# aimi-lab/robust-pose-estimator

Measured on AMD Instinct MI355X. Metric: stereo-pair pose solves/sec (640x512, 8 solver iters), higher is better.
Workload: dtype f32 (RAFT / geometry) + f64 (SE(3) solve), as the reference; 1 GPU; PoseNet.infer, 640x512 stereo frame pairs, 16 per GPU per step (RAFT batch 32), 12 GRU iters, lbfgs x8 SE(3) solve, weight heads on; frames_per_gpu=16, height=512, width=640, raft_iters=12, solver=lbfgs, solver_iters=8, parallelism=frames sharded x1

## Files before the change

### robust-pose-estimator_amd/csrc/conv_wino1d.hip

```cpp
#include "wino_common.h"
#include <type_traits>
#include <cstdlib>

#define W1_CO 64
#define W1_NT 64
#define W1_K 4
#define W1_ROW 8
#define W1_USTEP (W1_K * W1_CO * W1_ROW)
#define W1_RAWF 1536
#define W1_BIAS 1024u

struct W1P {
    const float* x; long long xbs;
    const float* wp; int cin, cout, coP, H, W;
    const float* bias; const float* add; long long abs_;
    float* out; long long obs; float* out2; long long o2bs;
    const float* hid; long long hbs; const float* z; long long zbs;
    int cgate, mode;
    int Hv, Wv;
};

__device__ __forceinline__ int row_swap(int r) { return ((r >> 2) ^ (r >> 3)) & 1; }

template <bool VERT, int CB, bool VALID = false>
__global__ __launch_bounds__(256, 2) void k_conv_wino1d(W1P P) {
    constexpr int TCO = 32 * CB, UT_STEP = W1_K * TCO * W1_ROW;
    __shared__ __attribute__((aligned(16))) float Us[3][UT_STEP];
    __shared__ __attribute__((aligned(16))) float Vs[2][W1_USTEP];
    __shared__ __attribute__((aligned(16))) float Rs[3][W1_RAWF];
    asm volatile("" :: "s"(P.x), "s"(P.wp), "s"(P.out), "s"(P.bias), "s"(P.xbs), "s"(P.obs), "s"(P.cin), "s"(P.cout), "s"(P.coP), "s"(P.H),
                 "s"(P.W), "s"(P.mode), "s"(P.cgate));
    asm volatile("" :: "s"(P.add), "s"(P.abs_), "s"(P.out2), "s"(P.o2bs), "s"(P.hid), "s"(P.hbs), "s"(P.z), "s"(P.zbs));
    const int tid = threadIdx.x, lane = tid & 63, wv = __builtin_amdgcn_readfirstlane(tid >> 6);
    const int ptx = (P.W + 15) / 16;
#ifndef WINO_NO_XCD
    const int pid = (gridDim.x & 7) == 0 ? (int)(blockIdx.x & 7) * (int)(gridDim.x >> 3) + (int)(blockIdx.x >> 3) : (int)blockIdx.x;
#else
    const int pid = blockIdx.x;
#endif
    const int x0 = (pid % ptx) * 16, y0 = (pid / ptx) * 16;
    const int co0 = blockIdx.y * TCO, bz = blockIdx.z;
    const int H = P.H, W = P.W, hw = H * W;
    const float* xb = P.x + (size_t)bz * P.xbs;
    const int nsteps = P.cin / W1_K;

    constexpr int LANES = VERT ? 40 : 48, RQ_CI = VERT ? 80 : 96, RQ_ROW = VERT ? 4 : 6;
    constexpr unsigned RSTRIDE = LANES * 16u;
    unsigned roff[2] = {0u, 0u};
    unsigned oob = 0;
    if (lane < LANES) {
#pragma unroll
        for (int j = 0; j < 2; ++j) {
            const int q = LANES * (2 * wv + j) + lane;
            const int ci = q / RQ_CI, rem = q - ci * RQ_CI, r = rem / RQ_ROW, cq = rem - r * RQ_ROW;
            int yy = VERT ? y0 - 2 + r : y0 + r, xx = VERT ? x0 + 4 * cq : x0 - 4 + 4 * cq;
            if (yy < 0 || yy >= H || xx < 0 || xx >= W) oob |= 1u << j;
            yy = yy < 0 ? 0 : (yy >= H ? H - 1 : yy); xx = xx < 0 ? 0 : (xx >= W ? W - 4 : xx);
            roff[j] = (unsigned)(ci * hw + yy * W + xx) * 4u + W1_BIAS - RSTRIDE * j;
        }
    }
    const bool border = VERT ? ((y0 < 2) | (y0 + 18 > H) | (x0 + 16 > W)) : ((y0 + 16 > H) | (x0 < 4) | (x0 + 20 > W));
    auto patch_raw = [&](int buf) {
        if (border) {
#pragma unroll
            for (int j = 0; j < 2; ++j)
                if ((oob >> j) & 1) *(f32x4*)&Rs[buf][4 * (LANES * (2 * wv + j) + lane)] = (f32x4){0.0f, 0.0f, 0.0f, 0.0f};
        }
    };
    const float* wslice = CB == 2 ? P.wp + (size_t)(co0 / W1_CO) * W1_USTEP + (size_t)(wv * 2) * 256
                                  : P.wp + (size_t)(co0 / W1_CO) * W1_USTEP + (size_t)wv * (W1_CO * W1_ROW) + (size_t)(co0 % W1_CO) * W1_ROW;
    const unsigned uoff = lane * 16u;
    const size_t wstep = (size_t)(P.coP / W1_CO) * W1_USTEP, rstep = (size_t)W1_K * hw;
    const unsigned us_base = lds_addr_of(&Us[0][0]) + (unsigned)wv * (CB == 2 ? 2048u : 1024u), rs_base = lds_addr_of(&Rs[0][0]) + (unsigned)(2 * wv) * RSTRIDE;
    const unsigned long long lane_mask = (1ull << LANES) - 1ull;
    auto dma_u = [&](const float* src, int buf) {
        if (CB == 2) dma16x2(src, uoff, us_base + (unsigned)buf * (UT_STEP * 4u));
        else dma16x1(src, uoff, us_base + (unsigned)buf * (UT_STEP * 4u));
    };
    auto dma_raw = [&](const float* src, int buf) { dma16x2_masked<RSTRIDE>(src, roff[0], roff[1], rs_base + (unsigned)buf * (W1_RAWF * 4u), lane_mask); };
    auto clamped = [&](int step) { return step < nsteps ? step : nsteps - 1; };
    const float* xsrc = xb - W1_BIAS / 4;

    const int t_src = VERT ? wv * (RQ_CI * 4) + (4 * (lane >> 4)) * 16 + (lane & 15) : wv * (RQ_CI * 4) + (lane >> 2) * 24 + 4 * (lane & 3) + 2;
    const int t_dst = (wv * W1_NT + lane) * W1_ROW, t_swap = row_swap(lane & 15);
    float d[8];
    f32x4 vlo, vhi;
    auto tr_read = [&](int rbuf) {
        const float* rp = &Rs[rbuf][t_src];
        if (VERT) {
#pragma unroll
            for (int k = 0; k < 8; ++k) d[k] = rp[16 * k];
        } else {
#pragma unroll
            for (int k = 0; k < 8; k += 2) { const float2 v = *(const float2*)(rp + k); d[k] = v.x; d[k + 1] = v.y; }
        }
    };
    auto tr_math = [&]() {
        const float a12 = fmaf(-4.25f, d[4], d[2] + d[6]), b12 = fmaf(-4.25f, d[3], d[1] + d[5]);
        const float a34 = fmaf(-1.25f, d[4], fmaf(0.25f, d[2], d[6])), b34 = fmaf(2.0f, d[5], fmaf(-2.5f, d[3], 0.5f * d[1]));
        const float a56 = fmaf(-5.0f, d[4], fmaf(4.0f, d[2], d[6])), b56 = fmaf(0.5f, d[5], fmaf(-2.5f, d[3], 2.0f * d[1]));
        vlo = (f32x4){fmaf(5.25f, d[4] - d[2], d[0] - d[6]), a12 + b12, a12 - b12, a34 + b34};
        vhi = (f32x4){a34 - b34, a56 + b56, a56 - b56, fmaf(5.25f, d[3] - d[5], d[7] - d[1])};
    };
    auto tr_store = [&](int vbuf) {
        *(f32x4*)&Vs[vbuf][t_dst + 4 * t_swap] = vlo;
        *(f32x4*)&Vs[vbuf][t_dst + 4 * (t_swap ^ 1)] = vhi;
    };

    f32x4 acc[8][CB][2];
#pragma unroll
    for (int p = 0; p < 8; ++p)
#pragma unroll
        for (int c = 0; c < CB; ++c)
#pragma unroll
            for (int t = 0; t < 2; ++t) acc[p][c][t] = (f32x4){0.0f, 0.0f, 0.0f, 0.0f};
    const int cw = wv >> 1, tw = wv & 1, li = lane & 15, lk = lane >> 4;
    float bi_[CB][4];
#pragma unroll
    for (int cb = 0; cb < CB; ++cb)
#pragma unroll
        for (int r = 0; r < 4; ++r) {
            const int co = co0 + cw * 16 * CB + cb * 16 + 4 * lk + r;
            bi_[cb][r] = P.bias ? P.bias[co < P.cout ? co : P.cout - 1] : 0.0f;
        }

    dma_u(wslice, 0); dma_raw(xsrc, 0); dma_raw(xsrc + (size_t)clamped(1) * rstep, 1);
    dma_u(wslice + (size_t)clamped(1) * wstep, 1); dma_raw(xsrc + (size_t)clamped(2) * rstep, 2);
    dma_u(wslice + (size_t)clamped(2) * wstep, 2);
    if (CB == 2) __builtin_amdgcn_s_waitcnt(0x0F76); else __builtin_amdgcn_s_waitcnt(0x0F74);
    patch_raw(0); patch_raw(1);
    __builtin_amdgcn_s_waitcnt(0xC07F);
    __builtin_amdgcn_s_barrier();
    tr_read(0); tr_math(); tr_store(0);
    __builtin_amdgcn_s_waitcnt(0xC07F);
    __builtin_amdgcn_s_barrier();
    dma_raw(xsrc + (size_t)clamped(3) * rstep, 0);
    const float* unext = wave_uniform(wslice + (size_t)clamped(3) * wstep);
    const float* rnext = wave_uniform(xsrc + (size_t)clamped(4) * rstep);
    const int sl = 4 * row_swap(li);
    const int aoff = (lk * TCO + cw * 16 * CB + li) * W1_ROW, boff = (lk * W1_NT + tw * 32 + li) * W1_ROW;
    f32x4 fa = *(const f32x4*)&Us[0][aoff + sl], fb0 = *(const f32x4*)&Vs[0][boff + sl], fb1 = *(const f32x4*)&Vs[0][boff + 16 * W1_ROW + sl];
    auto mfma_range = [&](int p0, int np, int cb, const f32x4& a, const f32x4& b0, const f32x4& b1) {
#pragma unroll
        for (int e = 0; e < np; ++e) {
            const int p = p0 + e;
            acc[p][cb][0] = __builtin_amdgcn_mfma_f32_16x16x4f32(a[p & 3], b0[p & 3], acc[p][cb][0], 0, 0, 0);
            acc[p][cb][1] = __builtin_amdgcn_mfma_f32_16x16x4f32(a[p & 3], b1[p & 3], acc[p][cb][1], 0, 0, 0);
        }
    };
    auto step = [&](auto ubc, auto curc, const int s) {
        constexpr int UB = decltype(ubc)::value, CUR = decltype(curc)::value, UB1 = (UB + 1) % 3, UB2 = (UB + 2) % 3;
        const float* ua = &Us[UB][aoff];
        const float* vb = &Vs[CUR][boff];
        f32x4 a_lo1 = fa;
        if (CB == 2) a_lo1 = *(const f32x4*)(ua + 16 * W1_ROW + sl);
        tr_read(UB1);
        __builtin_amdgcn_sched_barrier(0);
        if (CB == 2) mfma_range(0, 4, 0, fa, fb0, fb1); else mfma_range(0, 2, 0, fa, fb0, fb1);
        __builtin_amdgcn_sched_barrier(0);
        const f32x4 a_hi0 = *(const f32x4*)(ua + (sl ^ 4)), b_hi0 = *(const f32x4*)(vb + (sl ^ 4)), b_hi1 = *(const f32x4*)(vb + 16 * W1_ROW + (sl ^ 4));
        __builtin_amdgcn_sched_barrier(0);
        tr_math();
        __builtin_amdgcn_sched_barrier(0);
        if (CB == 2) mfma_range(0, 4, CB - 1, a_lo1, fb0, fb1); else mfma_range(2, 2, 0, fa, fb0, fb1);
        __builtin_amdgcn_sched_barrier(0);
        f32x4 a_hi1 = a_hi0;
        if (CB == 2) a_hi1 = *(const f32x4*)(ua + 16 * W1_ROW + (sl ^ 4));
        __builtin_amdgcn_sched_barrier(0);
        tr_store(CUR ^ 1);
        __builtin_amdgcn_sched_barrier(0);
        if (CB == 2) mfma_range(4, 4, 0, a_hi0, b_hi0, b_hi1); else mfma_range(4, 2, 0, a_hi0, b_hi0, b_hi1);
        __builtin_amdgcn_sched_barrier(0);
        if (CB == 2) __builtin_amdgcn_s_waitcnt(0x0F74); else __builtin_amdgcn_s_waitcnt(0x0F73);
        patch_raw(UB2);
        __builtin_amdgcn_s_waitcnt(0xC07F);
        __builtin_amdgcn_s_barrier();
        __builtin_amdgcn_sched_barrier(0);
        fa = *(const f32x4*)&Us[UB1][aoff + sl]; fb0 = *(const f32x4*)&Vs[CUR ^ 1][boff + sl]; fb1 = *(const f32x4*)&Vs[CUR ^ 1][boff + 16 * W1_ROW + sl];
        __builtin_amdgcn_sched_barrier(0);
#pragma unroll
        for (int e = 0; e < 2 * CB; ++e) {
            const int p = CB == 2 ? 4 + e : 6 + e;
            acc[p][CB - 1][0] = __builtin_amdgcn_mfma_f32_16x16x4f32(a_hi1[p & 3], b_hi0[p & 3], acc[p][CB - 1][0], 0, 0, 0);
            acc[p][CB - 1][1] = __builtin_amdgcn_mfma_f32_16x16x4f32(a_hi1[p & 3], b_hi1[p & 3], acc[p][CB - 1][1], 0, 0, 0);
            __builtin_amdgcn_sched_barrier(0);
            if (e == 0) { dma_u(unext, UB); if (s + 4 < nsteps) unext += wstep; }
            if (e == 1) { dma_raw(rnext, UB1); if (s + 5 < nsteps) rnext += rstep; }
            __builtin_amdgcn_sched_barrier(0);
        }
    };
    {
        typedef std::integral_constant<int, 0> I0; typedef std::integral_constant<int, 1> I1; typedef std::integral_constant<int, 2> I2;
        int s = 0;
        while (true) {
            step(I0{}, I0{}, s); if (++s == nsteps) break;
            step(I1{}, I1{}, s); if (++s == nsteps) break;
            step(I2{}, I0{}, s); if (++s == nsteps) break;
            step(I0{}, I1{}, s); if (++s == nsteps) break;
            step(I1{}, I0{}, s); if (++s == nsteps) break;
            step(I2{}, I1{}, s); if (++s == nsteps) break;
        }
    }
    __builtin_amdgcn_s_waitcnt(0x0F70);

    const int mode = P.mode, cg = P.cgate;
    const float* addb = P.add ? P.add + (size_t)bz * P.abs_ : nullptr;
    const float* hb = P.hid ? P.hid + (size_t)bz * P.hbs : nullptr;
    const float* zb = P.z ? P.z + (size_t)bz * P.zbs : nullptr;
    float* outb = P.out + (size_t)bz * P.obs;
    float* out2b = P.out2 ? P.out2 + (size_t)bz * P.o2bs : nullptr;
    float* tsc = &Us[0][wv * (CB == 2 ? 512 : 256)] + lk * 64;
    auto epilogue = [&](auto modec, auto fastc) {
        constexpr int MODE = decltype(modec)::value;
        constexpr bool FAST = decltype(fastc)::value;
        const bool rtile = co0 >= cg;
        constexpr int NB = 4 * CB, RU = 2;
        const f32x4 zero4 = {0.0f, 0.0f, 0.0f, 0.0f};
        auto where = [&](int tb, int& oy, int& ox) {
            const int tile = tw * 32 + tb * 16 + li;
            oy = VERT ? y0 + 4 * (tile >> 4) + (li >> 2) : y0 + (tile >> 2); ox = VERT ? x0 + 4 * (li & 3) : x0 + 4 * (tile & 3);
        };
        auto load_block = [&](int n, f32x4 (&av)[RU], f32x4 (&xv)[RU], f32x4 (&hv)[RU]) {
            const int tb = (n >> 1) / CB, cb = (n >> 1) % CB, r0 = RU * (n & 1);
            int oy, ox; where(tb, oy, ox);
            const bool pok = FAST || ((oy < H) & (ox < W));
            const size_t pxo = (size_t)oy * W + ox;
#pragma unroll
            for (int q = 0; q < RU; ++q) {
                const int co = co0 + cw * 16 * CB + cb * 16 + 4 * lk + r0 + q;
                const bool ok = FAST || (pok && co < P.cout);
                const size_t e0 = (size_t)co * hw + pxo;
                av[q] = (addb && ok) ? *(const f32x4*)(addb + e0) : zero4;
                xv[q] = hv[q] = zero4;
                if (MODE == RPE_CONV_GATE_ZR) { if (FAST ? rtile : (ok && co >= cg)) xv[q] = *(const f32x4*)(hb + e0 - (size_t)cg * hw); }
                else if (MODE == RPE_CONV_GATE_H) { if (ok) { xv[q] = *(const f32x4*)(zb + e0); hv[q] = *(const f32x4*)(hb + e0); } }
            }
        };
        auto finish_block = [&](int n, const f32x4 (&av)[RU], const f32x4 (&xv)[RU], const f32x4 (&hv)[RU]) {
            const int tb = (n >> 1) / CB, cb = (n >> 1) % CB, r0 = RU * (n & 1);
            int oy, ox; where(tb, oy, ox);
            const bool pok = FAST || ((oy < H) & (ox < W));
            const size_t pxo = (size_t)oy * W + ox;
            auto st4 = [&](float* p, size_t e, const float (&v)[4]) {
                f32x4 q4 = {v[0], v[1], v[2], v[3]};
                if (VALID && !FAST) {
#pragma unroll
                    for (int i = 0; i < 4; ++i) q4[i] = (oy < P.Hv && ox + i < P.Wv) ? q4[i] : 0.0f;
                }
                if (pok) *(f32x4*)(p + e) = q4;
            };
#pragma unroll
            for (int q = 0; q < RU; ++q) {
                const int r = r0 + q, co = co0 + cw * 16 * CB + cb * 16 + 4 * lk + r;
                if (!FAST && co >= P.cout) continue;
                float m[8];
#pragma unroll
                for (int p = 0; p < 8; ++p) m[p] = acc[p][cb][tb][r];
                const float s12 = m[1] + m[2], d12 = m[1] - m[2], s34 = m[3] + m[4], d34 = m[3] - m[4], s56 = m[5] + m[6], d56 = m[5] - m[6];
                float v[4] = {((m[0] + s12) + s34) + s56, fmaf(0.5f, d56, fmaf(2.0f, d34, d12)), fmaf(0.25f, s56, fmaf(4.0f, s34, s12)),
                              m[7] + fmaf(0.125f, d56, fmaf(8.0f, d34, d12))};
                if (VERT) {
#pragma unroll
                    for (int i = 0; i < 4; ++i) tsc[i * 16 + li] = v[i];
                    const f32x4 q = *(const f32x4*)&tsc[(li >> 2) * 16 + 4 * (li & 3)];
                    v[0] = q[0]; v[1] = q[1]; v[2] = q[2]; v[3] = q[3];
                }
                const size_t e0 = (size_t)co * hw + pxo;
                const float bi = bi_[cb][r];
#pragma unroll
                for (int i = 0; i < 4; ++i) v[i] = v[i] + av[q][i] + bi;
                if (MODE == RPE_CONV_GATE_ZR) {
                    float sg[4];
#pragma unroll
                    for (int i = 0; i < 4; ++i) sg[i] = sigmoid_f(v[i]);
                    if (FAST ? rtile : co >= cg) {
#pragma unroll
                        for (int i = 0; i < 4; ++i) sg[i] *= xv[q][i];
                        st4(out2b, e0 - (size_t)cg * hw, sg);
                    } else st4(outb, e0, sg);
                } else if (MODE == RPE_CONV_GATE_H) {
#pragma unroll
                    for (int i = 0; i < 4; ++i) v[i] = (1.0f - xv[q][i]) * hv[q][i] + xv[q][i] * tanh_f(v[i]);
                    st4(outb, e0, v);
                } else {
                    if (mode == RPE_CONV_RELU) {
#pragma unroll
                        for (int i = 0; i < 4; ++i) v[i] = v[i] < 0.0f ? 0.0f : v[i];
                    }
                    st4(outb, e0, v);
                    if (out2b) st4(out2b, e0, v);
                }
            }
        };
        f32x4 av_[2][RU], xv_[2][RU], hv_[2][RU];
        load_block(0, av_[0], xv_[0], hv_[0]);
#pragma unroll
        for (int n = 0; n < NB; ++n) {
            if (n + 1 < NB) load_block(n + 1, av_[(n + 1) & 1], xv_[(n + 1) & 1], hv_[(n + 1) & 1]);
            finish_block(n, av_[n & 1], xv_[n & 1], hv_[n & 1]);
        }
    };
    {
        typedef std::integral_constant<int, RPE_CONV_GATE_ZR> ZR; typedef std::integral_constant<int, RPE_CONV_GATE_H> GH; typedef std::integral_constant<int, -1> RT;
        typedef std::integral_constant<bool, true> Yes; typedef std::integral_constant<bool, false> No;
        const bool inside = (y0 + 16 <= (VALID ? P.Hv : H)) & (x0 + 16 <= (VALID ? P.Wv : W)) & (co0 + TCO <= P.cout);
        if (mode == RPE_CONV_GATE_ZR) { if (inside && (cg % TCO) == 0) epilogue(ZR{}, Yes{}); else epilogue(ZR{}, No{}); }
        else if (mode == RPE_CONV_GATE_H) { if (inside && CB == 1) epilogue(GH{}, Yes{}); else epilogue(GH{}, No{}); }
        else { if (inside) epilogue(RT{}, Yes{}); else epilogue(RT{}, No{}); }
    }
}

__global__ void k_wino1d_pack(const float* __restrict__ w, float* __restrict__ wp, int cout, int cin, int coP, long long total) {
    const long long e = (long long)blockIdx.x * blockDim.x + threadIdx.x;
    if (e >= total) return;
    const int slot = (int)(e & 7), col = (int)((e >> 3) & 63), cil = (int)((e >> 9) & 3);
    const int pos = (((slot >> 2) ^ row_swap(col & 15)) << 2) | (slot & 3);
    const long long rest = e >> 11;
    const int ncot = coP / W1_CO;
    const int co = (int)(rest % ncot) * W1_CO + col, ci = (int)(rest / ncot) * W1_K + cil;
    wp[e] = (co < cout && ci < cin) ? (float)wino1d_u(w + ((size_t)co * cin + ci) * 5, pos) : 0.0f;
}

extern "C" size_t rpe_conv_wino1d_packed_floats(int cout, int cin) {
    if (cout <= 0 || cin <= 0 || cin % W1_K) return 0;
    return (size_t)(cin / W1_K) * W1_K * W1_ROW * round_up(cout, W1_CO);
}

extern "C" int rpe_conv_wino1d_pack(const float* weight, int cout, int cin, float* packed, void* stream) {
    return launch_pack(k_wino1d_pack, weight, packed, cout, cin, W1_K, (long long)rpe_conv_wino1d_packed_floats(cout, cin), stream, round_up(cout, W1_CO));
}

static int conv_wino1d_launch(const rpe_conv_desc* d, int hv, int wv, void* stream) {
    if (!conv_desc_present(d)) return RPE_E_BADARG;
    const bool vert = d->kh == 5 && d->kw == 1, horiz = d->kh == 1 && d->kw == 5;
    if (!(vert || horiz) || !stride_is_1(d) || (d->cin % W1_K) || (d->w & 3)) return RPE_E_UNSUPPORTED;
    if (d->mode < RPE_CONV_LINEAR || d->mode > RPE_CONV_GATE_H || !conv_gate_args_ok(d)) return RPE_E_BADARG;
    if (!conv_no_encoder_epilogue(d)) return RPE_E_UNSUPPORTED;
    if (!aligned16(d->x, d->x_batch_stride) || !aligned16(d->packed, 0) || !aligned16(d->out, d->out_batch_stride) ||
        !aligned16(d->out2, d->out2_batch_stride) || !aligned16(d->add, d->add_batch_stride) || !aligned16(d->hidden, d->hidden_batch_stride) ||
        !aligned16(d->zgate, d->zgate_batch_stride)) return RPE_E_UNSUPPORTED;
    W1P P;
    fill_common(P, d, round_up(d->cout, W1_CO)); fill_gate(P, d);
    P.H = d->h; P.W = d->w; P.hid = d->hidden; P.hbs = d->hidden_batch_stride;
    P.Hv = hv; P.Wv = wv;
    const bool valid = hv != d->h || wv != d->w;
#ifndef WINO1D_SMALL_WG
#define WINO1D_SMALL_WG 768LL
#endif
    const long long small_wg = WINO1D_SMALL_WG;
    const unsigned gx = ceil_div(d->w, 16) * ceil_div(d->h, 16);
    if ((long long)gx * (P.coP / W1_CO) * d->b < small_wg) {
        const dim3 grid(gx, ceil_div(d->cout, 32), d->b);
        if (valid && vert) hipLaunchKernelGGL((k_conv_wino1d<true, 1, true>), grid, dim3(256), 0, (hipStream_t)stream, P);
        else if (valid) hipLaunchKernelGGL((k_conv_wino1d<false, 1, true>), grid, dim3(256), 0, (hipStream_t)stream, P);
        else if (vert) hipLaunchKernelGGL((k_conv_wino1d<true, 1>), grid, dim3(256), 0, (hipStream_t)stream, P);
        else hipLaunchKernelGGL((k_conv_wino1d<false, 1>), grid, dim3(256), 0, (hipStream_t)stream, P);
        return rpe_check_launch();
    }
    const dim3 grid(gx, P.coP / W1_CO, d->b);
    if (valid && vert) hipLaunchKernelGGL((k_conv_wino1d<true, 2, true>), grid, dim3(256), 0, (hipStream_t)stream, P);
    else if (valid) hipLaunchKernelGGL((k_conv_wino1d<false, 2, true>), grid, dim3(256), 0, (hipStream_t)stream, P);
    else if (vert) hipLaunchKernelGGL((k_conv_wino1d<true, 2>), grid, dim3(256), 0, (hipStream_t)stream, P);
    else hipLaunchKernelGGL((k_conv_wino1d<false, 2>), grid, dim3(256), 0, (hipStream_t)stream, P);
    return rpe_check_launch();
}

extern "C" int rpe_conv_wino1d(const rpe_conv_desc* d, void* stream) { return conv_wino1d_launch(d, d ? d->h : 0, d ? d->w : 0, stream); }

extern "C" int rpe_conv_wino1d_v(const rpe_conv_desc_v* dv, void* stream) {
    if (!dv || !conv_valid_extent_ok(dv)) return RPE_E_BADARG;
    return conv_wino1d_launch(&dv->d, dv->h_valid, dv->w_valid, stream);
}
```

Baseline: 251.6 pose solves/s.

## Add 128-output-channel wide tile variant for 1D Winograd 5-tap convolutions

Adds a WIDE template variant of the 1D Winograd conv kernel. Each block covers 128 output channels over a half-size spatial tile (8x16 or 16x8), so each input transform is reused across more output channels and the raw input traffic per block is halved. Only half the waves build the input transform each step, alternating between buffers. By default it is selected only for horizontal convs with cout divisible by 128 and enough workgroups, with an env override. The trade-off is fewer spatial tiles per block, more weight data in LDS per step, and less parallelism.

Result: no change. 253.8 pose solves/s, median of 6 (+0.9%).

```diff
diff --git a/robust-pose-estimator_amd/csrc/conv_wino1d.hip b/robust-pose-estimator_amd/csrc/conv_wino1d.hip
--- a/robust-pose-estimator_amd/csrc/conv_wino1d.hip
+++ b/robust-pose-estimator_amd/csrc/conv_wino1d.hip
@@ -22,36 +22,39 @@
 
 __device__ __forceinline__ int row_swap(int r) { return ((r >> 2) ^ (r >> 3)) & 1; }
 
-template <bool VERT, int CB, bool VALID = false>
+template <bool VERT, int CB, bool VALID = false, bool WIDE = false>
 __global__ __launch_bounds__(256, 2) void k_conv_wino1d(W1P P) {
-    constexpr int TCO = 32 * CB, UT_STEP = W1_K * TCO * W1_ROW;
+    static_assert(!WIDE || CB == 2, "the 128-channel class keeps the 32 x 32 wave");
+    constexpr int TCO = WIDE ? 128 : 32 * CB, NT = WIDE ? 32 : W1_NT, UT_STEP = W1_K * TCO * W1_ROW, VT_STEP = W1_K * NT * W1_ROW;
+    constexpr int RAWF = WIDE ? W1_RAWF / 2 : W1_RAWF;
+    constexpr int PH = (WIDE && !VERT) ? 8 : 16, PW = (WIDE && VERT) ? 8 : 16;
     __shared__ __attribute__((aligned(16))) float Us[3][UT_STEP];
-    __shared__ __attribute__((aligned(16))) float Vs[2][W1_USTEP];
-    __shared__ __attribute__((aligned(16))) float Rs[3][W1_RAWF];
+    __shared__ __attribute__((aligned(16))) float Vs[2][VT_STEP];
+    __shared__ __attribute__((aligned(16))) float Rs[3][RAWF];
     asm volatile("" :: "s"(P.x), "s"(P.wp), "s"(P.out), "s"(P.bias), "s"(P.xbs), "s"(P.obs), "s"(P.cin), "s"(P.cout), "s"(P.coP), "s"(P.H),
                  "s"(P.W), "s"(P.mode), "s"(P.cgate));
     asm volatile("" :: "s"(P.add), "s"(P.abs_), "s"(P.out2), "s"(P.o2bs), "s"(P.hid), "s"(P.hbs), "s"(P.z), "s"(P.zbs));
     const int tid = threadIdx.x, lane = tid & 63, wv = __builtin_amdgcn_readfirstlane(tid >> 6);
-    const int ptx = (P.W + 15) / 16;
+    const int ptx = (P.W + PW - 1) / PW;
 #ifndef WINO_NO_XCD
     const int pid = (gridDim.x & 7) == 0 ? (int)(blockIdx.x & 7) * (int)(gridDim.x >> 3) + (int)(blockIdx.x >> 3) : (int)blockIdx.x;
 #else
     const int pid = blockIdx.x;
 #endif
-    const int x0 = (pid % ptx) * 16, y0 = (pid / ptx) * 16;
+    const int x0 = (pid % ptx) * PW, y0 = (pid / ptx) * PH;
     const int co0 = blockIdx.y * TCO, bz = blockIdx.z;
     const int H = P.H, W = P.W, hw = H * W;
     const float* xb = P.x + (size_t)bz * P.xbs;
     const int nsteps = P.cin / W1_K;
 
-    constexpr int LANES = VERT ? 40 : 48, RQ_CI = VERT ? 80 : 96, RQ_ROW = VERT ? 4 : 6;
+    constexpr int LANES = VERT ? 40 : 48, NJ = WIDE ? 1 : 2, RQ_CI = LANES * NJ, RQ_ROW = VERT ? (WIDE ? 2 : 4) : 6;
     constexpr unsigned RSTRIDE = LANES * 16u;
     unsigned roff[2] = {0u, 0u};
     unsigned oob = 0;
     if (lane < LANES) {
 #pragma unroll
-        for (int j = 0; j < 2; ++j) {
-            const int q = LANES * (2 * wv + j) + lane;
+        for (int j = 0; j < NJ; ++j) {
+            const int q = LANES * (NJ * wv + j) + lane;
             const int ci = q / RQ_CI, rem = q - ci * RQ_CI, r = rem / RQ_ROW, cq = rem - r * RQ_ROW;
             int yy = VERT ? y0 - 2 + r : y0 + r, xx = VERT ? x0 + 4 * cq : x0 - 4 + 4 * cq;
             if (yy < 0 || yy >= H || xx < 0 || xx >= W) oob |= 1u << j;
@@ -59,37 +62,46 @@
             roff[j] = (unsigned)(ci * hw + yy * W + xx) * 4u + W1_BIAS - RSTRIDE * j;
         }
     }
-    const bool border = VERT ? ((y0 < 2) | (y0 + 18 > H) | (x0 + 16 > W)) : ((y0 + 16 > H) | (x0 < 4) | (x0 + 20 > W));
+    const bool border = VERT ? ((y0 < 2) | (y0 + PH + 2 > H) | (x0 + PW > W)) : ((y0 + PH > H) | (x0 < 4) | (x0 + 20 > W));
     auto patch_raw = [&](int buf) {
         if (border) {
 #pragma unroll
-            for (int j = 0; j < 2; ++j)
-                if ((oob >> j) & 1) *(f32x4*)&Rs[buf][4 * (LANES * (2 * wv + j) + lane)] = (f32x4){0.0f, 0.0f, 0.0f, 0.0f};
-        }
-    };
-    const float* wslice = CB == 2 ? P.wp + (size_t)(co0 / W1_CO) * W1_USTEP + (size_t)(wv * 2) * 256
+            for (int j = 0; j < NJ; ++j)
+                if ((oob >> j) & 1) *(f32x4*)&Rs[buf][4 * (LANES * (NJ * wv + j) + lane)] = (f32x4){0.0f, 0.0f, 0.0f, 0.0f};
+        }
+    };
+    const float* wslice = WIDE    ? P.wp + (size_t)(co0 / W1_CO) * W1_USTEP + (size_t)(wv * 4) * 256
+                        : CB == 2 ? P.wp + (size_t)(co0 / W1_CO) * W1_USTEP + (size_t)(wv * 2) * 256
                                   : P.wp + (size_t)(co0 / W1_CO) * W1_USTEP + (size_t)wv * (W1_CO * W1_ROW) + (size_t)(co0 % W1_CO) * W1_ROW;
     const unsigned uoff = lane * 16u;
     const size_t wstep = (size_t)(P.coP / W1_CO) * W1_USTEP, rstep = (size_t)W1_K * hw;
-    const unsigned us_base = lds_addr_of(&Us[0][0]) + (unsigned)wv * (CB == 2 ? 2048u : 1024u), rs_base = lds_addr_of(&Rs[0][0]) + (unsigned)(2 * wv) * RSTRIDE;
+    constexpr unsigned UWAVE = WIDE ? 4096u : CB == 2 ? 2048u : 1024u;
+    const unsigned us_base = lds_addr_of(&Us[0][0]) + (unsigned)wv * UWAVE, rs_base = lds_addr_of(&Rs[0][0]) + (unsigned)(NJ * wv) * RSTRIDE;
     const unsigned long long lane_mask = (1ull << LANES) - 1ull;
     auto dma_u = [&](const float* src, int buf) {
-        if (CB == 2) dma16x2(src, uoff, us_base + (unsigned)buf * (UT_STEP * 4u));
+        if (WIDE) dma16x4(src, uoff, us_base + (unsigned)buf * (UT_STEP * 4u));
+        else if (CB == 2) dma16x2(src, uoff, us_base + (unsigned)buf * (UT_STEP * 4u));
         else dma16x1(src, uoff, us_base + (unsigned)buf * (UT_STEP * 4u));
     };
-    auto dma_raw = [&](const float* src, int buf) { dma16x2_masked<RSTRIDE>(src, roff[0], roff[1], rs_base + (unsigned)buf * (W1_RAWF * 4u), lane_mask); };
+    auto dma_raw = [&](const float* src, int buf) {
+        if (WIDE) dma16x1_masked(src, roff[0], rs_base + (unsigned)buf * (RAWF * 4u), lane_mask);
+        else dma16x2_masked<RSTRIDE>(src, roff[0], roff[1], rs_base + (unsigned)buf * (RAWF * 4u), lane_mask);
+    };
     auto clamped = [&](int step) { return step < nsteps ? step : nsteps - 1; };
     const float* xsrc = xb - W1_BIAS / 4;
 
-    const int t_src = VERT ? wv * (RQ_CI * 4) + (4 * (lane >> 4)) * 16 + (lane & 15) : wv * (RQ_CI * 4) + (lane >> 2) * 24 + 4 * (lane & 3) + 2;
-    const int t_dst = (wv * W1_NT + lane) * W1_ROW, t_swap = row_swap(lane & 15);
+    const int t_ci = WIDE ? 2 * (wv & 1) + (lane >> 5) : wv, t_tile = WIDE ? (lane & 31) : lane;
+    const int t_src = VERT ? t_ci * (RQ_CI * 4) + (4 * (WIDE ? t_tile >> 3 : t_tile >> 4)) * PW + (t_tile & (PW - 1))
+                           : t_ci * (RQ_CI * 4) + (t_tile >> 2) * 24 + 4 * (t_tile & 3) + 2;
+    const int t_dst = (t_ci * NT + t_tile) * W1_ROW, t_swap = row_swap(t_tile & 15);
+    const bool t_even = !WIDE || (wv >> 1) == 0;
     float d[8];
     f32x4 vlo, vhi;
     auto tr_read = [&](int rbuf) {
         const float* rp = &Rs[rbuf][t_src];
         if (VERT) {
 #pragma unroll
-            for (int k = 0; k < 8; ++k) d[k] = rp[16 * k];
+            for (int k = 0; k < 8; ++k) d[k] = rp[PW * k];
         } else {
 #pragma unroll
             for (int k = 0; k < 8; k += 2) { const float2 v = *(const float2*)(rp + k); d[k] = v.x; d[k + 1] = v.y; }
@@ -114,7 +126,7 @@
         for (int c = 0; c < CB; ++c)
 #pragma unroll
             for (int t = 0; t < 2; ++t) acc[p][c][t] = (f32x4){0.0f, 0.0f, 0.0f, 0.0f};
-    const int cw = wv >> 1, tw = wv & 1, li = lane & 15, lk = lane >> 4;
+    const int cw = WIDE ? wv : wv >> 1, tw = WIDE ? 0 : wv & 1, li = lane & 15, lk = lane >> 4;
     float bi_[CB][4];
 #pragma unroll
     for (int cb = 0; cb < CB; ++cb)
@@ -127,18 +139,20 @@
     dma_u(wslice, 0); dma_raw(xsrc, 0); dma_raw(xsrc + (size_t)clamped(1) * rstep, 1);
     dma_u(wslice + (size_t)clamped(1) * wstep, 1); dma_raw(xsrc + (size_t)clamped(2) * rstep, 2);
     dma_u(wslice + (size_t)clamped(2) * wstep, 2);
-    if (CB == 2) __builtin_amdgcn_s_waitcnt(0x0F76); else __builtin_amdgcn_s_waitcnt(0x0F74);
+    if (WIDE) __builtin_amdgcn_s_waitcnt(0x0F79);
+    else if (CB == 2) __builtin_amdgcn_s_waitcnt(0x0F76); else __builtin_amdgcn_s_waitcnt(0x0F74);
     patch_raw(0); patch_raw(1);
     __builtin_amdgcn_s_waitcnt(0xC07F);
     __builtin_amdgcn_s_barrier();
-    tr_read(0); tr_math(); tr_store(0);
+    if (t_even) { tr_read(0); tr_math(); tr_store(0); }
     __builtin_amdgcn_s_waitcnt(0xC07F);
     __builtin_amdgcn_s_barrier();
     dma_raw(xsrc + (size_t)clamped(3) * rstep, 0);
     const float* unext = wave_uniform(wslice + (size_t)clamped(3) * wstep);
     const float* rnext = wave_uniform(xsrc + (size_t)clamped(4) * rstep);
     const int sl = 4 * row_swap(li);
-    const int aoff = (lk * TCO + cw * 16 * CB + li) * W1_ROW, boff = (lk * W1_NT + tw * 32 + li) * W1_ROW;
+    const int aoff = WIDE ? ((cw >> 1) * (W1_K * W1_CO) + lk * W1_CO + (cw & 1) * 32 + li) * W1_ROW : (lk * TCO + cw * 16 * CB + li) * W1_ROW;
+    const int boff = (lk * NT + tw * 32 + li) * W1_ROW;
     f32x4 fa = *(const f32x4*)&Us[0][aoff + sl], fb0 = *(const f32x4*)&Vs[0][boff + sl], fb1 = *(const f32x4*)&Vs[0][boff + 16 * W1_ROW + sl];
     auto mfma_range = [&](int p0, int np, int cb, const f32x4& a, const f32x4& b0, const f32x4& b1) {
 #pragma unroll
@@ -152,26 +166,28 @@
         constexpr int UB = decltype(ubc)::value, CUR = decltype(curc)::value, UB1 = (UB + 1) % 3, UB2 = (UB + 2) % 3;
         const float* ua = &Us[UB][aoff];
         const float* vb = &Vs[CUR][boff];
+        const bool build = CUR == 1 ? t_even : (!WIDE || !t_even);
         f32x4 a_lo1 = fa;
         if (CB == 2) a_lo1 = *(const f32x4*)(ua + 16 * W1_ROW + sl);
-        tr_read(UB1);
+        if (build) tr_read(UB1);
         __builtin_amdgcn_sched_barrier(0);
         if (CB == 2) mfma_range(0, 4, 0, fa, fb0, fb1); else mfma_range(0, 2, 0, fa, fb0, fb1);
         __builtin_amdgcn_sched_barrier(0);
         const f32x4 a_hi0 = *(const f32x4*)(ua + (sl ^ 4)), b_hi0 = *(const f32x4*)(vb + (sl ^ 4)), b_hi1 = *(const f32x4*)(vb + 16 * W1_ROW + (sl ^ 4));
         __builtin_amdgcn_sched_barrier(0);
-        tr_math();
+        if (build) tr_math();
         __builtin_amdgcn_sched_barrier(0);
         if (CB == 2) mfma_range(0, 4, CB - 1, a_lo1, fb0, fb1); else mfma_range(2, 2, 0, fa, fb0, fb1);
         __builtin_amdgcn_sched_barrier(0);
         f32x4 a_hi1 = a_hi0;
         if (CB == 2) a_hi1 = *(const f32x4*)(ua + 16 * W1_ROW + (sl ^ 4));
         __builtin_amdgcn_sched_barrier(0);
-        tr_store(CUR ^ 1);
+        if (build) tr_store(CUR ^ 1);
         __builtin_amdgcn_sched_barrier(0);
         if (CB == 2) mfma_range(4, 4, 0, a_hi0, b_hi0, b_hi1); else mfma_range(4, 2, 0, a_hi0, b_hi0, b_hi1);
         __builtin_amdgcn_sched_barrier(0);
-        if (CB == 2) __builtin_amdgcn_s_waitcnt(0x0F74); else __builtin_amdgcn_s_waitcnt(0x0F73);
+        if (WIDE) __builtin_amdgcn_s_waitcnt(0x0F75);
+        else if (CB == 2) __builtin_amdgcn_s_waitcnt(0x0F74); else __builtin_amdgcn_s_waitcnt(0x0F73);
         patch_raw(UB2);
         __builtin_amdgcn_s_waitcnt(0xC07F);
         __builtin_amdgcn_s_barrier();
@@ -209,7 +225,7 @@
     const float* zb = P.z ? P.z + (size_t)bz * P.zbs : nullptr;
     float* outb = P.out + (size_t)bz * P.obs;
     float* out2b = P.out2 ? P.out2 + (size_t)bz * P.o2bs : nullptr;
-    float* tsc = &Us[0][wv * (CB == 2 ? 512 : 256)] + lk * 64;
+    float* tsc = &Us[0][wv * (UWAVE / 4)] + lk * 64;
     auto epilogue = [&](auto modec, auto fastc) {
         constexpr int MODE = decltype(modec)::value;
         constexpr bool FAST = decltype(fastc)::value;
@@ -218,7 +234,8 @@
         const f32x4 zero4 = {0.0f, 0.0f, 0.0f, 0.0f};
         auto where = [&](int tb, int& oy, int& ox) {
             const int tile = tw * 32 + tb * 16 + li;
-            oy = VERT ? y0 + 4 * (tile >> 4) + (li >> 2) : y0 + (tile >> 2); ox = VERT ? x0 + 4 * (li & 3) : x0 + 4 * (tile & 3);
+            if (WIDE && VERT) { oy = y0 + 8 * tb + (li >> 1); ox = x0 + 4 * (li & 1); }
+            else { oy = VERT ? y0 + 4 * (tile >> 4) + (li >> 2) : y0 + (tile >> 2); ox = VERT ? x0 + 4 * (li & 3) : x0 + 4 * (tile & 3); }
         };
         auto load_block = [&](int n, f32x4 (&av)[RU], f32x4 (&xv)[RU], f32x4 (&hv)[RU]) {
             const int tb = (n >> 1) / CB, cb = (n >> 1) % CB, r0 = RU * (n & 1);
@@ -261,8 +278,8 @@
                               m[7] + fmaf(0.125f, d56, fmaf(8.0f, d34, d12))};
                 if (VERT) {
 #pragma unroll
-                    for (int i = 0; i < 4; ++i) tsc[i * 16 + li] = v[i];
-                    const f32x4 q = *(const f32x4*)&tsc[(li >> 2) * 16 + 4 * (li & 3)];
+                    for (int i = 0; i < 4; ++i) tsc[WIDE ? (4 * (li >> 3) + i) * 8 + (li & 7) : i * 16 + li] = v[i];
+                    const f32x4 q = *(const f32x4*)&tsc[WIDE ? (li >> 1) * 8 + 4 * (li & 1) : (li >> 2) * 16 + 4 * (li & 3)];
                     v[0] = q[0]; v[1] = q[1]; v[2] = q[2]; v[3] = q[3];
                 }
                 const size_t e0 = (size_t)co * hw + pxo;
@@ -303,7 +320,7 @@
     {
         typedef std::integral_constant<int, RPE_CONV_GATE_ZR> ZR; typedef std::integral_constant<int, RPE_CONV_GATE_H> GH; typedef std::integral_constant<int, -1> RT;
         typedef std::integral_constant<bool, true> Yes; typedef std::integral_constant<bool, false> No;
-        const bool inside = (y0 + 16 <= (VALID ? P.Hv : H)) & (x0 + 16 <= (VALID ? P.Wv : W)) & (co0 + TCO <= P.cout);
+        const bool inside = (y0 + PH <= (VALID ? P.Hv : H)) & (x0 + PW <= (VALID ? P.Wv : W)) & (co0 + TCO <= P.cout);
         if (mode == RPE_CONV_GATE_ZR) { if (inside && (cg % TCO) == 0) epilogue(ZR{}, Yes{}); else epilogue(ZR{}, No{}); }
         else if (mode == RPE_CONV_GATE_H) { if (inside && CB == 1) epilogue(GH{}, Yes{}); else epilogue(GH{}, No{}); }
         else { if (inside) epilogue(RT{}, Yes{}); else epilogue(RT{}, No{}); }
@@ -349,6 +366,26 @@
 #endif
     const long long small_wg = WINO1D_SMALL_WG;
     const unsigned gx = ceil_div(d->w, 16) * ceil_div(d->h, 16);
+    int wide = 0;
+#ifndef WINO1D_NO_CO128
+#ifndef WINO1D_CO128_WG
+#define WINO1D_CO128_WG 512LL
+#endif
+    const unsigned gw = vert ? ceil_div(d->w, 8) * ceil_div(d->h, 16) : ceil_div(d->w, 16) * ceil_div(d->h, 8);
+    if (d->cout % 128 == 0) {
+        const char* env = getenv("RPE_WINO1D_CO128");
+        const int force = (env && (env[0] == '0' || env[0] == '1') && !env[1]) ? env[0] - '0' : -1;
+        wide = force >= 0 ? force : (!vert && (long long)gx * (P.coP / W1_CO) * d->b >= small_wg && (long long)gw * (d->cout / 128) * d->b >= WINO1D_CO128_WG);
+    }
+    if (wide) {
+        const dim3 grid(gw, d->cout / 128, d->b);
+        if (valid && vert) hipLaunchKernelGGL((k_conv_wino1d<true, 2, true, true>), grid, dim3(256), 0, (hipStream_t)stream, P);
+        else if (valid) hipLaunchKernelGGL((k_conv_wino1d<false, 2, true, true>), grid, dim3(256), 0, (hipStream_t)stream, P);
+        else if (vert) hipLaunchKernelGGL((k_conv_wino1d<true, 2, false, true>), grid, dim3(256), 0, (hipStream_t)stream, P);
+        else hipLaunchKernelGGL((k_conv_wino1d<false, 2, false, true>), grid, dim3(256), 0, (hipStream_t)stream, P);
+        return rpe_check_launch();
+    }
+#endif
     if ((long long)gx * (P.coP / W1_CO) * d->b < small_wg) {
         const dim3 grid(gx, ceil_div(d->cout, 32), d->b);
         if (valid && vert) hipLaunchKernelGGL((k_conv_wino1d<true, 1, true>), grid, dim3(256), 0, (hipStream_t)stream, P);
```
